# gorjanradevski/revisiting-spatial-temporal-layouts

Measured on AMD Instinct MI355X. Metric: clips/s STLT forward (T=32, N_obj=7, d=768), higher is better.
Workload: dtype f32; 1 GPU; cfg2: STLT forward, T=32, N=7, d=768, H=12, 4+8 layers, 174 classes; per_gpu_batch=1024, global_batch=1024, parallelism=batch-shard x1, no collective, cls_only_last_spatial=True

## Files before the change

revisiting-spatial-temporal-layouts_amd/csrc/gemm.hip:

```cpp
#include <cstdlib>
#include <type_traits>
#include "common.h"

namespace {

constexpr int BM = 256, BN = 128, BK = 32;
constexpr int GEMM_WAVES = 8;
constexpr int GEMM_LOADERS = 4;
constexpr int GEMM_THREADS = 64 * (GEMM_WAVES + GEMM_LOADERS);
constexpr int NSTAGE = 3;
constexpr int STAGE_FLOATS = (BM + BN) * BK;

typedef __attribute__((address_space(3))) void* lds_void_ptr;
typedef const __attribute__((address_space(1))) void* glb_void_ptr;

#ifndef STLT_GEMM_ABLATE
#define STLT_GEMM_ABLATE 0
#endif
__device__ __forceinline__ float half_wave_sum(float x) {
  x += __shfl_xor(x, 1, 64);
  x += __shfl_xor(x, 2, 64);
  x += __shfl_xor(x, 4, 64);
  x += __shfl_xor(x, 8, 64);
  x += __shfl_xor(x, 16, 64);
  return x;
}

struct SkPlan { int dp_rounds; int P[9]; int S[8]; };
struct SkNone {};
template <bool B, class T> auto karg(const T& t) { if constexpr (B) return t; else return SkNone{}; }

template <int ACT, bool STAMP, bool TA, bool TB, bool ADD, bool SK, bool GROUP = false>
__global__ __launch_bounds__(GEMM_THREADS, 3) void gemm_nt_kernel(const float* __restrict__ X, int64_t ldx,
                                                                  const float* __restrict__ W, int64_t ldw,
                                                                  const float* __restrict__ bias,
                                                                  const float* __restrict__ R, int64_t ldr,
                                                                  float* __restrict__ Y, int64_t ldy,
                                                                  int64_t slab_stride, int M, int N, int K,
                                                                  int tiles_m, int tiles_n, int n_split,
                                                                  float* __restrict__ partials,
                                                                  unsigned long long* __restrict__ dbg,
                                                                  const std::conditional_t<SK, SkPlan, SkNone> plan_in,
                                                                  const std::conditional_t<GROUP, StltGemmGroup, SkNone> grp_in,
                                                                  const std::conditional_t<ACT == STLT_ACT_GELU_BWD, StltGemmEpi, SkNone> epi_in) {
  SkPlan plan{}; StltGemmGroup grp{}; StltGemmEpi epi{};
  if constexpr (SK) plan = plan_in;
  if constexpr (GROUP) grp = grp_in;
  if constexpr (ACT == STLT_ACT_GELU_BWD) epi = epi_in;
  static_assert(!GROUP || SK, "grouped launches are stream-K launches");
  static_assert(ACT != STLT_ACT_GELU_BWD || (ADD && !GROUP), "the fused GELU backward reads u through the add-source");
  constexpr int NBIAS = 2;
  __shared__ __attribute__((aligned(16))) float smem[NSTAGE * STAGE_FLOATS + NBIAS * BN];

  const int tid = threadIdx.x;
  const int lane = tid & 63;
  const int wave = __builtin_amdgcn_readfirstlane(tid >> 6);
  const int wm = wave >> 1, wn = wave & 1;
  const int lr = lane & 31, lh = lane >> 5;
  const int nk_total = K / BK;
  int nk = GROUP ? 1 : nk_total / n_split;
  const int n_tiles = GROUP ? grp.tile_base[grp.n] : tiles_m * tiles_n * n_split;

  const int G = gridDim.x;
  int v = blockIdx.x;
  if ((G & 7) == 0) v = (blockIdx.x & 7) * (G >> 3) + (blockIdx.x >> 3);
  constexpr int GROUP_M = 4;
  const bool grouped = !SK && n_split == 1 && (G & 7) == 0;
  const int g_xcd = blockIdx.x & 7, g_local = blockIdx.x >> 3, g_gx = G >> 3;
  const int g_rounds = (n_tiles + G - 1) / G;
  int my_tiles, sk_first = 0, sk_kt0 = 0, sk_tail = 0;
  const bool hy = SK && plan.dp_rounds > 0;
  const int hy_R = hy ? plan.dp_rounds : 0;
  int hy_steps = 0;
  int g_p0 = 0, g_first = 0, g_nk_last = 1, g_total = 0;
  if constexpr (GROUP) {
    const int total = grp.step_base[grp.n];
    const int S = (total + G - 1) / G;
    const int s0 = v * S;
    if (s0 >= total) return;
    const int s1 = s0 + S < total ? s0 + S : total;
    while (grp.step_base[g_p0 + 1] <= s0) ++g_p0;
    const int nk0 = grp.p[g_p0].nk;
    const int lt0 = (s0 - grp.step_base[g_p0]) / nk0;
    sk_kt0 = s0 - grp.step_base[g_p0] - lt0 * nk0;
    g_first = grp.tile_base[g_p0] + lt0;
    int p1 = g_p0;
    while (grp.step_base[p1 + 1] <= s1 - 1) ++p1;
    g_nk_last = grp.p[p1].nk;
    const int lt1 = (s1 - 1 - grp.step_base[p1]) / g_nk_last;
    my_tiles = grp.tile_base[p1] + lt1 - g_first + 1;
    sk_tail = s1 - (grp.step_base[p1] + lt1 * g_nk_last);
    g_total = s1 - s0;
  } else
  if (hy) {
    const int e = plan.P[g_xcd + 1];
    const int s0 = plan.P[g_xcd] + g_local * plan.S[g_xcd];
    const int s1 = s0 + plan.S[g_xcd] < e ? s0 + plan.S[g_xcd] : e;
    int sk_tiles = 0;
    if (s0 < s1) {
      sk_first = s0 / nk;
      sk_kt0 = s0 - sk_first * nk;
      const int last = (s1 - 1) / nk;
      sk_tiles = last - sk_first + 1;
      sk_tail = s1 - last * nk;
      hy_steps = s1 - s0;
    }
    my_tiles = hy_R + sk_tiles;
  } else if (SK) {
    const int total = n_tiles * nk;
    const int S = (total + G - 1) / G;
    const int s0 = v * S;
    if (s0 >= total) return;
    const int s1 = s0 + S < total ? s0 + S : total;
    sk_first = s0 / nk;
    sk_kt0 = s0 - sk_first * nk;
// ... 183 lines not shown
      }
    }
  };
  if (wave >= GEMM_WAVES) {
    int l_it = 0, l_kt = kt_begin(0), l_stage = 0;
    bool l_fresh = true;
    auto l_step = [&]() {
      if ((STLT_GEMM_ABLATE & 32) ? l_fresh : (l_kt == 0 || l_fresh)) { dma_set_tile(l_it); l_fresh = false; }
      const int src_kt = (STLT_GEMM_ABLATE & 32) ? 0 : l_kt;
#pragma unroll
      for (int u = 0; u < NV; ++u) {
        issue_dma_part(0, src_kt, l_stage, u);
        issue_dma_part(1, src_kt, l_stage, u);
        issue_dma_part(2, src_kt, l_stage, u);
      }
      if (++l_kt == nk) { ++l_it; l_kt = kt_begin(l_it); if (!(STLT_GEMM_ABLATE & 32)) l_fresh = true; }
      if (++l_stage == NSTAGE) l_stage = 0;
    };
    dma_bias(0);
    l_step();
    if (total_steps > 1) {
      l_step();
      asm volatile("s_waitcnt vmcnt(12)" ::: "memory");
    } else {
      asm volatile("s_waitcnt vmcnt(0)" ::: "memory");
    }
    __builtin_amdgcn_s_barrier();
    int w_it = 0, w_kt = kt_begin(0);
    for (int step = 0; step < total_steps; ++step) {
      if (!GROUP && w_kt == nk - 1 && w_it + 1 < my_tiles) dma_bias(w_it + 1);
      if (!(STLT_GEMM_ABLATE & 1) && step + 2 < total_steps) {
        l_step();
        if (!(STLT_GEMM_ABLATE & 8)) asm volatile("s_waitcnt vmcnt(12)" ::: "memory");
      } else {
        asm volatile("s_waitcnt vmcnt(0)" ::: "memory");
      }
      __builtin_amdgcn_s_barrier();
      if (!GROUP && ++w_kt == nk) { ++w_it; w_kt = kt_begin(w_it); }
    }
    return;
  }
  f32x16 acc[2][2];
  auto init_acc = [&](int it, bool zero) {
    if (bias && !TB && !zero) {
      const float* src = bias_lds + (it & 1) * BN + wn * 64 + 4 * lh;
#pragma unroll
      for (int b = 0; b < 2; ++b)
#pragma unroll
        for (int q = 0; q < 4; ++q) {
          const f32x4 v = *reinterpret_cast<const f32x4*>(src + b * 32 + 8 * q);
#pragma unroll
          for (int j = 0; j < 4; ++j) { acc[0][b][4 * q + j] = v[j]; acc[1][b][4 * q + j] = v[j]; }
        }
    } else {
#pragma unroll
      for (int a = 0; a < 2; ++a)
#pragma unroll
        for (int b = 0; b < 2; ++b)
#pragma unroll
          for (int r = 0; r < 16; ++r) acc[a][b][r] = 0.f;
    }
  };

  auto mfma_chunk = [&](const Frags& f) {
#pragma unroll
    for (int e = 0; e < 4; ++e) {
      acc[0][0] = __builtin_amdgcn_mfma_f32_32x32x2f32(f.b0[e], f.a0[e], acc[0][0], 0, 0, 0);
      acc[0][1] = __builtin_amdgcn_mfma_f32_32x32x2f32(f.b1[e], f.a0[e], acc[0][1], 0, 0, 0);
      acc[1][0] = __builtin_amdgcn_mfma_f32_32x32x2f32(f.b0[e], f.a1[e], acc[1][0], 0, 0, 0);
      acc[1][1] = __builtin_amdgcn_mfma_f32_32x32x2f32(f.b1[e], f.a1[e], acc[1][1], 0, 0, 0);
    }
  };

  __builtin_amdgcn_s_barrier();
  init_acc(0, SK && !seg_complete(0));
  Frags fa = read_frags(0, 0), fb;

  int c_it = 0, c_kt = kt_begin(0);
  if constexpr (GROUP) nk = grp.p[g_p0].nk;
  int stage = 0;
  constexpr bool RES_PF = ADD && !SK && !TA && !TB;
  f32x4 rpf[RES_PF ? 8 : 1];
  bool rpf_ok = false;
  unsigned long long t_acc[6] = {0, 0, 0, 0, 0, 0}, t_prev = 0;
#define GSTAMP(k) do { if (STAMP) { __builtin_amdgcn_sched_barrier(0); unsigned long long t_now = __builtin_amdgcn_s_memtime(); __builtin_amdgcn_s_waitcnt(0xC07F); t_acc[k] += t_now - t_prev; t_prev = t_now; __builtin_amdgcn_sched_barrier(0); } } while (0)
  if (STAMP) { t_prev = __builtin_amdgcn_s_memtime(); __builtin_amdgcn_s_waitcnt(0xC07F); }
  for (int step = 0; step < total_steps; ++step) {
    const int next_stage = stage + 1 == NSTAGE ? 0 : stage + 1;
    if constexpr (RES_PF) {
      if (c_kt == nk - 1) {
        int m0, n0, split;
        tile_origin(c_it, m0, n0, split);
        rpf_ok = (m0 + BM <= M) && (n0 + BN <= N) && (ldr & 3) == 0 && ((uintptr_t)R & 15) == 0;
        if (rpf_ok) {
          const float* rrow = R + (int64_t)(m0 + wm * 64 + lr) * ldr + n0;
#pragma unroll
          for (int h = 0; h < 8; ++h) rpf[h] = *reinterpret_cast<const f32x4*>(rrow + wn * 64 + (h >> 2) * 32 + 8 * (h & 3) + 4 * lh);
        }
      }
    }
    fb = read_frags(stage, 1);
    mfma_chunk(fa);
    fa = read_frags(stage, 2);
    mfma_chunk(fb);
    fb = read_frags(stage, 3);
    mfma_chunk(fa);
    if (STAMP) asm volatile("" :: "v"(acc[0][0][0]), "v"(acc[1][1][15]));
    GSTAMP(0);
    asm volatile("s_waitcnt lgkmcnt(0)" ::: "memory");
    GSTAMP(1);
    __builtin_amdgcn_s_barrier();
    GSTAMP(2);
    GSTAMP(3);
    if (step + 1 < total_steps) fa = read_frags(next_stage, 0);
    mfma_chunk(fb);
    if (STAMP) asm volatile("" :: "v"(acc[0][0][0]), "v"(acc[1][1][15]));
    GSTAMP(4);
    stage = next_stage;

    if (++c_kt == nk || (SK && step == total_steps - 1)) {
      int m0, n0, split;
      tile_origin(c_it, m0, n0, split);
      if constexpr (GROUP) {
        int pi, lt;
        group_tile(c_it, pi, lt);
        Y = grp.p[pi].c; ldy = grp.p[pi].ldc; R = grp.p[pi].r; ldr = grp.p[pi].ldr; M = grp.p[pi].M; N = grp.p[pi].N;
      }
      float* Yt = Y + (int64_t)split * slab_stride;
      const bool partial = SK && !seg_complete(c_it);
      const bool vec_ok = (m0 + BM <= M) && (n0 + BN <= N) && (ldy & 3) == 0 && ((uintptr_t)Yt & 15) == 0 &&
                          (!ADD || ((ldr & 3) == 0 && ((uintptr_t)R & 15) == 0));
      auto t_row = [&](int a) { return TA ? wm * 64 + 2 * lr + a : wm * 64 + a * 32 + lr; };
      auto t_col4 = [&](int g) { return TB ? wn * 64 + 16 * (g >> 1) + 8 * lh + 4 * (g & 1) : wn * 64 + (g >> 2) * 32 + 8 * (g & 3) + 4 * lh; };
      auto group = [&](int a, int g) {
        f32x4 v;
#pragma unroll
        for (int j = 0; j < 4; ++j)
          v[j] = TB ? acc[a][j & 1][4 * (g >> 1) + 2 * (g & 1) + (j >> 1)] : acc[a][g >> 2][4 * (g & 3) + j];
        return v;
      };
      if (partial) {
        float* P = partials + (size_t)(2 * v + (c_it == hy_R ? 0 : 1)) * (BM * BN);
#pragma unroll
        for (int a = 0; a < 2; ++a)
#pragma unroll
          for (int g = 0; g < 8; ++g) *reinterpret_cast<f32x4*>(P + t_row(a) * BN + t_col4(g)) = group(a, g);
      } else if (ACT == STLT_ACT_GELU_BWD && vec_ok) {
        const uint64_t key = stlt_drop_key(epi.dr, epi.site);
        float* cs_row = epi.cs_part + ((size_t)(m0 / BM) * 16 + wm) * (size_t)N + n0;
        uint64_t drow[2];
#pragma unroll
        for (int a = 0; a < 2; ++a) drow[a] = epi.drop_rows ? (uint64_t)epi.drop_rows[m0 + t_row(a)] : (uint64_t)(m0 + t_row(a));
        constexpr int GB = 2;
#pragma unroll
        for (int hf = 0; hf < 8 / GB; ++hf) {
          f32x4 uv[2][GB];
#pragma unroll
          for (int a = 0; a < 2; ++a)
#pragma unroll
            for (int q = 0; q < GB; ++q) uv[a][q] = *reinterpret_cast<const f32x4*>(R + (int64_t)(m0 + t_row(a)) * ldr + n0 + t_col4(hf * GB + q));
#pragma unroll
          for (int q = 0; q < GB; ++q) {
            const int g = hf * GB + q;
            f32x4 cs = {0.f, 0.f, 0.f, 0.f};
#pragma unroll
            for (int a = 0; a < 2; ++a) {
              const f32x4 val = gelu_bwd4(group(a, g), uv[a][q], epi, key, drow[a] * (uint64_t)N + (uint64_t)(n0 + t_col4(g)));
              *reinterpret_cast<f32x4*>(Yt + (int64_t)(m0 + t_row(a)) * ldy + n0 + t_col4(g)) = val;
              cs += val;
            }
#pragma unroll
            for (int j = 0; j < 4; ++j) cs[j] = half_wave_sum(cs[j]);
            if (lr == 0) {
              *reinterpret_cast<f32x4*>(cs_row + t_col4(g)) = cs;
#pragma unroll
              for (int k = 1; k < 4; ++k) *reinterpret_cast<f32x4*>(cs_row + (size_t)(4 * k) * N + t_col4(g)) = f32x4{0.f, 0.f, 0.f, 0.f};
            }
          }
        }
      } else if (ACT == STLT_ACT_GELU_BWD) {
        const uint64_t key = stlt_drop_key(epi.dr, epi.site);
        float* cs_row = epi.cs_part + ((size_t)(m0 / BM) * 16 + wm) * (size_t)N;
#pragma unroll
        for (int g = 0; g < 8; ++g) {
          f32x4 cs = {0.f, 0.f, 0.f, 0.f};
          const int n = n0 + t_col4(g);
#pragma unroll
          for (int a = 0; a < 2; ++a) {
            const int m = m0 + t_row(a);
            const f32x4 acc4 = group(a, g);
            if (m < M) {
              const uint64_t drow1 = epi.drop_rows ? (uint64_t)epi.drop_rows[m] : (uint64_t)m;
#pragma unroll
              for (int j = 0; j < 4; ++j) {
                if (n + j < N) {
                  float v = acc4[j];
                  if (epi.dr.thr) v = stlt_keep_k(epi.dr.thr, key, drow1 * (uint64_t)N + (uint64_t)(n + j)) ? v * epi.dr.scale : 0.f;
                  v *= gelu_grad_epilogue(R[(int64_t)m * ldr + n + j]);
                  Yt[(int64_t)m * ldy + n + j] = v;
                  cs[j] += v;
                }
              }
            }
          }
#pragma unroll
          for (int j = 0; j < 4; ++j) cs[j] = half_wave_sum(cs[j]);
          if (lr == 0) {
#pragma unroll
            for (int j = 0; j < 4; ++j)
              if (n + j < N) {
                cs_row[n + j] = cs[j];
#pragma unroll
                for (int k = 1; k < 4; ++k) cs_row[(size_t)(4 * k) * N + n + j] = 0.f;
              }
          }
        }
      } else if (vec_ok) {
#pragma unroll
        for (int a = 0; a < 2; ++a) {
          const int m = m0 + t_row(a);
          float* yrow = Yt + (int64_t)m * ldy + n0;
          const float* rrow = ADD ? R + (int64_t)m * ldr + n0 : nullptr;
          constexpr int RB = 8;
          f32x4 rv[ADD ? RB : 1];
#pragma unroll
          for (int g = 0; g < 8; ++g) {
            if (ADD && g % RB == 0) {
              if (RES_PF && a == 0 && rpf_ok) {
#pragma unroll
                for (int h = 0; h < RB; ++h) rv[ADD ? h : 0] = rpf[RES_PF ? h : 0];
              } else {
#pragma unroll
                for (int h = 0; h < RB; ++h) rv[ADD ? h : 0] = *reinterpret_cast<const f32x4*>(rrow + t_col4(g + h));
              }
            }
            f32x4 val = group(a, g);
            if (ADD) val += rv[ADD ? g % RB : 0];
#pragma unroll
            for (int j = 0; j < 4; ++j) {
              if (ACT == STLT_ACT_GELU) val[j] = gelu_epilogue(val[j]);
              if (ACT == STLT_ACT_RELU) val[j] = fmaxf(val[j], 0.f);
            }
            if (STLT_GEMM_ABLATE & 16) asm volatile("" :: "v"(val));
            else *reinterpret_cast<f32x4*>(yrow + t_col4(g)) = val;
          }
        }
      } else {
#pragma unroll
        for (int a = 0; a < 2; ++a) {
          const int m = m0 + t_row(a);
#pragma unroll
          for (int g = 0; g < 8; ++g) {
            const int n = n0 + t_col4(g);
            const f32x4 val = group(a, g);
            float* yp = Yt + (int64_t)m * ldy + n;
            const float* rp = ADD ? R + (int64_t)m * ldr + n : nullptr;
#pragma unroll
            for (int j = 0; j < 4; ++j) {
              float x = val[j];
              if (m < M && n + j < N) {
                if (ADD) x += rp[j];
                if (ACT == STLT_ACT_GELU) x = gelu_epilogue(x);
                if (ACT == STLT_ACT_RELU) x = fmaxf(x, 0.f);
                yp[j] = x;
              }
            }
          }
        }
      }
      if (c_it + 1 < my_tiles) init_acc(c_it + 1, SK && !seg_complete(c_it + 1));
      ++c_it;
      c_kt = kt_begin(c_it);
      if constexpr (GROUP) {
        if (c_it < my_tiles) { int pi, lt; group_tile(c_it, pi, lt); nk = grp.p[pi].nk; }
      }
      GSTAMP(5);
    }
  }
  if (dbg && tid == 0) {
    dbg[4 * blockIdx.x + 1] = __builtin_amdgcn_s_memrealtime();
    dbg[4 * (size_t)gridDim.x + (size_t)gridDim.x * GEMM_WAVES * 6 + 1024 + 2 * blockIdx.x + 1] = __builtin_amdgcn_s_memtime();
  }
  if (STAMP && dbg && lane == 0) {
    unsigned long long* o = dbg + 4 * (size_t)gridDim.x + ((size_t)blockIdx.x * GEMM_WAVES + wave) * 6;
    for (int k = 0; k < 6; ++k) o[k] = t_acc[k];
  }
#undef GSTAMP
}


constexpr int FIXUP_CHUNKS = 16;
template <int ACT>
__global__ __launch_bounds__(256) void gemm_fixup_kernel(const float* __restrict__ partials, int S, int nk,
                                                         const float* __restrict__ bias, const float* __restrict__ R,
                                                         int64_t ldr, float* __restrict__ Y, int64_t ldy, int M, int N,
                                                         int tiles_m, int tiles_n, int G, const SkPlan plan, const StltGemmEpi epi) {
  __shared__ float cs_red[8][BN];
  const int t = blockIdx.x / FIXUP_CHUNKS, chunk = blockIdx.x - t * FIXUP_CHUNKS;
  const int lo = t * nk, hi = lo + nk;
  const bool hy = plan.dp_rounds > 0;
  const int gx = G >> 3;
  auto wg_of = [&](int s) {
    if (!hy) return s / S;
    int x = 0;
    while (x < 7 && s >= plan.P[x + 1]) ++x;
    return x * gx + (s - plan.P[x]) / plan.S[x];
  };
  auto start_of = [&](int v) {
    if (!hy) return v * S;
    const int x = v / gx;
    return plan.P[x] + (v - x * gx) * plan.S[x];
  };
  const int v_first = wg_of(lo), v_last = wg_of(hi - 1);
  if (v_first == v_last) return;
  int m0, n0;
  if (hy) {
    constexpr int GROUP_M = 4;
    const int p = plan.dp_rounds * G + t;
    const int band = p / (GROUP_M * tiles_n), w = p - band * (GROUP_M * tiles_n);
    const int rows = tiles_m - band * GROUP_M < GROUP_M ? tiles_m - band * GROUP_M : GROUP_M;
    const int tn_g = w / rows;
    m0 = (band * GROUP_M + (w - tn_g * rows)) * BM;
    n0 = tn_g * BN;
  } else {
    const int tm = t / tiles_n;
    m0 = tm * BM;
    n0 = (t - tm * tiles_n) * BN;
  }
  const int c4 = (threadIdx.x & 31) * 4;
  float bv[4];
#pragma unroll
  for (int e = 0; e < 4; ++e) bv[e] = (bias && n0 + c4 + e < N) ? bias[n0 + c4 + e] : 0.f;
  const int r_end = (chunk + 1) * (BM / FIXUP_CHUNKS);
  const uint64_t key = ACT == STLT_ACT_GELU_BWD ? stlt_drop_key(epi.dr, epi.site) : 0ull;
  f32x4 cs = {0.f, 0.f, 0.f, 0.f};
  for (int rr = chunk * (BM / FIXUP_CHUNKS) + (threadIdx.x >> 5); rr < r_end; rr += 8) {
    const int m = m0 + rr;
    if (m >= M) break;
    f32x4 acc = {0.f, 0.f, 0.f, 0.f};
    for (int v = v_first; v <= v_last; ++v) {
      if (hy && start_of(v) >= plan.P[v / gx + 1]) continue;
      const size_t slot = (size_t)(2 * v + (start_of(v) >= lo ? 0 : 1));
      acc += *reinterpret_cast<const f32x4*>(partials + slot * (BM * BN) + rr * BN + c4);
    }
    const uint64_t drow = (ACT == STLT_ACT_GELU_BWD && epi.drop_rows) ? (uint64_t)epi.drop_rows[m] : (uint64_t)m;
#pragma unroll
    for (int e = 0; e < 4; ++e) {
      const int n = n0 + c4 + e;
      if (n < N) {
        float val = acc[e] + bv[e];
        if (ACT == STLT_ACT_GELU_BWD) {
          if (epi.dr.thr) val = stlt_keep_k(epi.dr.thr, key, drow * (uint64_t)N + (uint64_t)n) ? val * epi.dr.scale : 0.f;
          val *= gelu_grad_epilogue(R[(int64_t)m * ldr + n]);
          cs[e] += val;
        } else if (R) {
          val += R[(int64_t)m * ldr + n];
        }
        if (ACT == STLT_ACT_GELU) val = gelu_epilogue(val);
        if (ACT == STLT_ACT_RELU) val = fmaxf(val, 0.f);
        Y[(int64_t)m * ldy + n] = val;
      }
    }
  }
  if (ACT == STLT_ACT_GELU_BWD) {
#pragma unroll
    for (int e = 0; e < 4; ++e) cs_red[threadIdx.x >> 5][c4 + e] = cs[e];
    __syncthreads();
    if (threadIdx.x < BN && n0 + (int)threadIdx.x < N) {
      float tsum = 0.f;
#pragma unroll
// ... 291 lines not shown
  if (act == STLT_ACT_GELU_BWD) {
    if (!epi_in || !epi.cs_part || !r || transA || (!transB && !on_copy) || n_split != 1 || bias)
      return stlt_set_error(STLT_EINVAL, "gemm: the fused GELU backward is the dX layout with u as the add-source and a column-sum buffer");
  }
  if (M < 0 || N <= 0 || K <= 0) return stlt_set_error(STLT_EINVAL, "gemm: bad shape (M=%lld N=%lld K=%lld)", (long long)M, (long long)N, (long long)K);
  const bool base_off = (((uintptr_t)a | (uintptr_t)b) & 15) != 0;
  if (K % BK != 0 || lda % 4 != 0 || ldb % 4 != 0 || base_off) {
    if ((n_split != 1 || act == STLT_ACT_GELU_BWD) && base_off && K % BK == 0 && lda % 4 == 0 && ldb % 4 == 0)
      return stlt_set_error(STLT_EINVAL, "gemm: a split product / the fused GELU backward needs %s 16-byte aligned", ((uintptr_t)a & 15) ? "a" : "b");
    if (n_split != 1 || act == STLT_ACT_GELU_BWD)
      return stlt_set_error(STLT_EINVAL, "gemm: a split product / the fused GELU backward needs K=%lld to be a multiple of %d and pitches that are multiples of 4", (long long)K, BK);
    return launch_gemm_any(transA, transB, a, lda, b, ldb, bias, r, ldr, c, ldc, M, N, K, act, s);
  }
  if (lda % 4 != 0 || ldb % 4 != 0 || (r && ldr < N) || ldc < N || lda < (transA ? M : K) || ldb < (transB ? N : K))
    return stlt_set_error(STLT_EINVAL, "gemm: bad leading dimension (lda=%lld ldb=%lld ldc=%lld)", (long long)lda, (long long)ldb, (long long)ldc);
  if (M > 0x7fffff00LL || N > 0x7fffff00LL || (bias && N > 0x3fffff00LL)) return stlt_set_error(STLT_EINVAL, "gemm: M/N too large");
  if (lda > 0x3fffffLL || ldb > 0x3fffffLL)
    return stlt_set_error(STLT_EINVAL, "gemm: row pitch too large (lda=%lld ldb=%lld, at most 4194303 floats)", (long long)lda, (long long)ldb);
  if (act != STLT_ACT_NONE && act != STLT_ACT_GELU && act != STLT_ACT_RELU && act != STLT_ACT_GELU_BWD) return stlt_set_error(STLT_EINVAL, "gemm: unknown activation %d", act);
  if (n_split < 1 || (K / BK) % n_split != 0) return stlt_set_error(STLT_EINVAL, "gemm: n_split=%d must divide K/32=%lld", n_split, (long long)(K / BK));
  if (transA && !transB) return stlt_set_error(STLT_EINVAL, "gemm: the (transA, !transB) layout is not built");
  if (n_split > 1 && (bias || act != STLT_ACT_NONE || r)) return stlt_set_error(STLT_EINVAL, "gemm: a split product takes no bias / activation / add-source");
  if ((transA || transB) && ((act != STLT_ACT_NONE && act != STLT_ACT_GELU_BWD) || bias)) return stlt_set_error(STLT_EINVAL, "gemm: bias/activation only with the forward (NT) layout");
  if (r && act != STLT_ACT_NONE && act != STLT_ACT_GELU_BWD) return stlt_set_error(STLT_EINVAL, "gemm: an add-source excludes an activation");
  if (M == 0) return 0;
  const int64_t tiles_m = (M + BM - 1) / BM, tiles_n = (N + BN - 1) / BN;
  if (tiles_m * tiles_n * n_split > 0x7fffffffLL) return stlt_set_error(STLT_EINVAL, "gemm: too many tiles");
  int64_t n_wg = tiles_m * tiles_n * n_split;
  if (n_wg > n_cu()) n_wg = n_cu();
  StltProfScope ps(STLT_K_GEMM, s);
  stlt_prof_add_flops(2.0 * (double)M * (double)N * (double)K);
  stlt_prof_note("gemm%s M=%lld N=%lld K=%lld act=%d%s tile=256x128 tiles=%lld", transA ? "(dW)" : (transB ? "(dX)" : (on_copy ? "(dX on the Wt copy)" : "")), (long long)M, (long long)N, (long long)K, act,
                 r ? "+R" : "", (long long)(tiles_m * tiles_n));
  const dim3 block(GEMM_THREADS);
  const int64_t n_tiles = tiles_m * tiles_n, nk = K / BK;
  const int64_t rounds = (n_tiles + n_cu() - 1) / n_cu();
  const double fill = (double)n_tiles / (double)(rounds * n_cu());
  static const double sk_fill = [] { const char* e = getenv("STLT_GEMM_SK_FILL"); return e ? atof(e) : 0.9; }();
  bool weighted = false;
  if (xcd_weights() && n_split == 1 && t_gemm_scratch && fill >= sk_fill && n_tiles >= 4 * (int64_t)n_cu() && n_tiles * nk < 0x7fffffffLL) {
    SkPlan probe{};
    int64_t tail = 0;
    weighted = make_sk_plan(n_tiles, nk, n_cu() < STLT_GEMM_SK_MAX_WG ? n_cu() : STLT_GEMM_SK_MAX_WG, xcd_weights(), true, probe, tail);
  }
  if (n_split == 1 && t_gemm_scratch && (fill < sk_fill || weighted) && n_tiles * nk < 0x7fffffffLL && !g_stlt_debug_buf) {
    int64_t G = n_cu() < STLT_GEMM_SK_MAX_WG ? n_cu() : STLT_GEMM_SK_MAX_WG;
    if (n_tiles * nk < 4 * G) G = (n_tiles * nk + 3) / 4;
    if (t_gemm_scratch_bytes >= (size_t)(2 * G) * BM * BN * sizeof(float)) {
      const int S = (int)((n_tiles * nk + G - 1) / G);
      dim3 grid((unsigned)G);
      float* P = t_gemm_scratch;
      stlt_prof_note("stream-K wg=%lld ksteps/wg=%d (+fix-up)", (long long)G, S);
      static const bool hybrid_on = [] { const char* e = getenv("STLT_GEMM_HYBRID"); return e ? atoi(e) != 0 : true; }();
      SkPlan plan{};
      int64_t fix_tiles = n_tiles;
      if (hybrid_on && G == n_cu()) {
        int64_t tail = 0;
        if (make_sk_plan(n_tiles, nk, G, xcd_weights(), weighted, plan, tail)) fix_tiles = tail;
        else plan = SkPlan{};
      }
#define LAUNCH_SK(ACTV, TAV, TBV, ADDV) hipLaunchKernelGGL((gemm_nt_kernel<ACTV, false, TAV, TBV, ADDV, true>), grid, block, 0, s, a, lda, b, ldb, bias, r, ldr, c, ldc, slab_stride, (int)M, (int)N, (int)K, (int)tiles_m, (int)tiles_n, 1, P, nullptr, plan, SkNone{}, karg<(ACTV) == STLT_ACT_GELU_BWD>(epi))
      if (transA) { if (r) LAUNCH_SK(STLT_ACT_NONE, true, true, true); else LAUNCH_SK(STLT_ACT_NONE, true, true, false); }
      else if (transB && act == STLT_ACT_GELU_BWD) LAUNCH_SK(STLT_ACT_GELU_BWD, false, true, true);
      else if (transB) { if (r) LAUNCH_SK(STLT_ACT_NONE, false, true, true); else LAUNCH_SK(STLT_ACT_NONE, false, true, false); }
      else if (act == STLT_ACT_GELU_BWD) LAUNCH_SK(STLT_ACT_GELU_BWD, false, false, true);
      else if (r) LAUNCH_SK(STLT_ACT_NONE, false, false, true);
      else if (act == STLT_ACT_GELU) LAUNCH_SK(STLT_ACT_GELU, false, false, false);
      else if (act == STLT_ACT_RELU) LAUNCH_SK(STLT_ACT_RELU, false, false, false);
      else LAUNCH_SK(STLT_ACT_NONE, false, false, false);
#undef LAUNCH_SK
      if (int e = stlt_check_launch("gemm_nt_kernel(stream-k)")) return e;
      dim3 fgrid((unsigned)(fix_tiles * FIXUP_CHUNKS)), fblock(256);
#define FIX(ACTV) hipLaunchKernelGGL((gemm_fixup_kernel<ACTV>), fgrid, fblock, 0, s, P, S, (int)nk, bias, r, ldr, c, ldc, (int)M, (int)N, (int)tiles_m, (int)tiles_n, (int)G, plan, epi)
      if (act == STLT_ACT_GELU_BWD) FIX(STLT_ACT_GELU_BWD);
      else if (act == STLT_ACT_GELU) FIX(STLT_ACT_GELU);
      else if (act == STLT_ACT_RELU) FIX(STLT_ACT_RELU);
      else FIX(STLT_ACT_NONE);
#undef FIX
      return stlt_check_launch("gemm_fixup_kernel");
    }
  }
  dim3 grid((unsigned)n_wg);
  stlt_prof_note("wg=%lld rounds=%lld ksteps=%lld split=%d", (long long)n_wg, (long long)((tiles_m * tiles_n * n_split + n_wg - 1) / n_wg), (long long)(nk / n_split), n_split);
#define LAUNCH(ACTV, STAMPV, TAV, TBV, ADDV) hipLaunchKernelGGL((gemm_nt_kernel<ACTV, STAMPV, TAV, TBV, ADDV, false>), grid, block, 0, s, a, lda, b, ldb, bias, r, ldr, c, ldc, slab_stride, (int)M, (int)N, (int)K, (int)tiles_m, (int)tiles_n, n_split, (float*)nullptr, g_stlt_debug_buf, SkNone{}, SkNone{}, karg<(ACTV) == STLT_ACT_GELU_BWD>(epi))
  if (transA) { if (r) LAUNCH(STLT_ACT_NONE, false, true, true, true); else LAUNCH(STLT_ACT_NONE, false, true, true, false); }
  else if (transB && act == STLT_ACT_GELU_BWD) LAUNCH(STLT_ACT_GELU_BWD, false, false, true, true);
  else if (transB) { if (r) LAUNCH(STLT_ACT_NONE, false, false, true, true); else LAUNCH(STLT_ACT_NONE, false, false, true, false); }
  else if (act == STLT_ACT_GELU_BWD) LAUNCH(STLT_ACT_GELU_BWD, false, false, false, true);
  else if (r && g_stlt_debug_buf && getenv("STLT_GEMM_STAMP")) LAUNCH(STLT_ACT_NONE, true, false, false, true);
  else if (r) LAUNCH(STLT_ACT_NONE, false, false, false, true);
  else if (g_stlt_debug_buf && getenv("STLT_GEMM_STAMP")) LAUNCH(STLT_ACT_NONE, true, false, false, false);
  else if (act == STLT_ACT_GELU) LAUNCH(STLT_ACT_GELU, false, false, false, false);
  else if (act == STLT_ACT_RELU) LAUNCH(STLT_ACT_RELU, false, false, false, false);
  else LAUNCH(STLT_ACT_NONE, false, false, false, false);
#undef LAUNCH
  return stlt_check_launch("gemm_nt_kernel");
}

bool stlt_gemm_has_scratch() { return t_gemm_scratch != nullptr && t_gemm_scratch_bytes >= STLT_GEMM_SCRATCH_BYTES; }
float* stlt_gemm_scratch_ptr(size_t* bytes) { *bytes = t_gemm_scratch ? t_gemm_scratch_bytes : 0; return t_gemm_scratch; }

int launch_weight_grad_group(const StltWeightGradItem* items, int n_items, hipStream_t s) {
  if (!items || n_items < 1 || n_items > STLT_GEMM_GROUP_MAX) return stlt_set_error(STLT_EINVAL, "weight_grad_group: 1..%d items", STLT_GEMM_GROUP_MAX);
  if (!stlt_gemm_has_scratch()) return stlt_set_error(STLT_EWORKSPACE, "weight_grad_group: no stream-K scratch lent (StltGemmScratch)");
  StltGemmGroup grp{};
  int64_t tiles = 0, steps = 0;
  double flops = 0.0;
  int n = 0;
  for (int i = 0; i < n_items; ++i) {
    const StltWeightGradItem& it = items[i];
    if (!it.g_w || it.rows == 0) continue;
    if (!it.dy || !it.x || it.n_out <= 0 || it.k_in <= 0 || it.rows < 0 || it.rows % BK != 0 || it.n_out % 4 != 0 || it.k_in % 4 != 0)
      return stlt_set_error(STLT_EINVAL, "weight_grad_group: item %d: rows=%lld must be a multiple of %d, n_out=%lld / k_in=%lld multiples of 4", i,
                            (long long)it.rows, BK, (long long)it.n_out, (long long)it.k_in);
    if (it.n_out > 0x3fffffLL || it.k_in > 0x3fffffLL || it.rows > 0x7fffff00LL) return stlt_set_error(STLT_EINVAL, "weight_grad_group: item too large");
    if (const char* off = stlt_first_unaligned16({{"dy", it.dy}, {"x", it.x}}))
      return stlt_set_error(STLT_EINVAL, "weight_grad_group: item %d: %s must be 16-byte aligned", i, off);
    const int64_t tm = (it.n_out + BM - 1) / BM, tn = (it.k_in + BN - 1) / BN;
    StltGemmProblem& q = grp.p[n];
    q.a = it.dy; q.lda = (int)it.n_out; q.b = it.x; q.ldb = (int)it.k_in; q.r = it.g_w; q.ldr = (int)it.k_in; q.c = it.g_w; q.ldc = (int)it.k_in;
    q.M = (int)it.n_out; q.N = (int)it.k_in; q.nk = (int)(it.rows / BK); q.tiles_n = (int)tn;
    grp.tile_base[n] = (int)tiles;
    grp.step_base[n] = (int)steps;
    tiles += tm * tn;
    steps += tm * tn * (it.rows / BK);
    if (tiles > 0x3fffffffLL || steps > 0x3fffffffLL) return stlt_set_error(STLT_EINVAL, "weight_grad_group: too many k-steps");
    flops += 2.0 * (double)it.n_out * (double)it.k_in * (double)it.rows;
    ++n;
  }
  if (n == 0) return 0;
  grp.n = n;
  for (int i = n; i <= STLT_GEMM_GROUP_MAX; ++i) { grp.tile_base[i] = (int)tiles; grp.step_base[i] = (int)steps; }
  int64_t G = n_cu() < STLT_GEMM_SK_MAX_WG ? n_cu() : STLT_GEMM_SK_MAX_WG;
  if (steps < 4 * G) G = (steps + 3) / 4;
  const int S = (int)((steps + G - 1) / G);
  StltProfScope ps(STLT_K_GEMM, s);
  stlt_prof_add_flops(flops);
  stlt_prof_note("gemm(dW group) products=%d tiles=%lld ksteps=%lld tile=256x128 stream-K wg=%lld ksteps/wg=%d (+fix-up)", n, (long long)tiles, (long long)steps, (long long)G, S);
  float* P = t_gemm_scratch;
  hipLaunchKernelGGL((gemm_nt_kernel<STLT_ACT_NONE, false, true, true, true, true, true>), dim3((unsigned)G), dim3(GEMM_THREADS), 0, s,
                     (const float*)nullptr, (int64_t)0, (const float*)nullptr, (int64_t)0, (const float*)nullptr, (const float*)nullptr, (int64_t)0,
                     (float*)nullptr, (int64_t)0, (int64_t)0, 0, 0, BK, 0, 0, 1, P, (unsigned long long*)nullptr, SkPlan{}, grp, SkNone{});
  if (int e = stlt_check_launch("gemm_nt_kernel(grouped stream-k)")) return e;
  hipLaunchKernelGGL(gemm_fixup_group_kernel, dim3((unsigned)(tiles * FIXUP_CHUNKS)), dim3(256), 0, s, P, S, grp);
  return stlt_check_launch("gemm_fixup_group_kernel");
}

StltGemmScratch::StltGemmScratch(void* p, size_t bytes) : prev_(t_gemm_scratch), prev_bytes_(t_gemm_scratch_bytes) {
  t_gemm_scratch = static_cast<float*>(p);
  t_gemm_scratch_bytes = p ? bytes : 0;
}
StltGemmScratch::~StltGemmScratch() {
  t_gemm_scratch = prev_;
  t_gemm_scratch_bytes = prev_bytes_;
}
StltGemmWgCap::StltGemmWgCap(int n) : prev_(t_gemm_wg_cap) { t_gemm_wg_cap = n > 0 ? (n + 7) / 8 * 8 : 0; }
StltGemmWgCap::~StltGemmWgCap() { t_gemm_wg_cap = prev_; }
void stlt_gemm_set_scratch_impl(void* p, size_t bytes) {
  t_gemm_scratch = static_cast<float*>(p);
  t_gemm_scratch_bytes = p ? bytes : 0;
}

int launch_reduce_slabs(const float* slabs, int64_t stride, int n_slabs, float* dst, int64_t n, int accumulate, hipStream_t s) {
  if (!slabs || !dst || n_slabs < 1) return stlt_set_error(STLT_EINVAL, "reduce_slabs: bad arguments");
  if (n == 0) return 0;
  if (accumulate) { int err = 0; if (reduce_defer_take(slabs, stride, n_slabs, dst, nullptr, nullptr, 1, n, s, &err)) return err; }
  const bool off16 = (((uintptr_t)slabs | (uintptr_t)dst) & 15) != 0 || (n_slabs > 1 && stride % 4 != 0);
  if (off16 && (n + 15) / 16 > 0x7fffffffLL) return stlt_set_error(STLT_EINVAL, "reduce_slabs: n=%lld is too large for slabs / dst off a 16-byte boundary", (long long)n);
  if ((n_slabs > 32 && n <= 16384) || off16) {
    stlt_prof_note("reduce n=%lld slabs=%d tall blocks=%lld", (long long)n, n_slabs, (long long)((n + 15) / 16));
    hipLaunchKernelGGL(reduce_tall_kernel, dim3((unsigned)((n + 15) / 16)), dim3(256), 0, s, slabs, stride, n_slabs, dst, n, accumulate);
    return stlt_check_launch("reduce_tall_kernel");
  }
  int64_t blocks = (n + 1023) / 1024;
  if (blocks > 2048) blocks = 2048;
  stlt_prof_note("reduce n=%lld slabs=%d blocks=%lld", (long long)n, n_slabs, (long long)blocks);
  hipLaunchKernelGGL(reduce_slabs_kernel, dim3((unsigned)blocks), dim3(256), 0, s, slabs, stride, n_slabs, dst, n, accumulate);
  return stlt_check_launch("reduce_slabs_kernel");
// ... 41 lines not shown
```

Baseline: 9901 clips/s.

## Overlap GEMM epilogue stores with next tile's MFMA at tile boundaries

Adds a skewed boundary path for forward whole-tile GEMM launches. The last k-step of a tile and the first k-step of the next are merged, so the epilogue (bias/residual add, activation, stores) of each accumulator half is interleaved with MFMAs of the other half. Scheduling group barriers pin the instruction order for some variants. The aim is to hide the serial epilogue cost between tiles, at the price of much more complex control flow, register pressure from residual prefetch, and 32-bit address arithmetic limits. It also extends the timestamp instrumentation with per-epilogue counters.

```diff
diff --git a/revisiting-spatial-temporal-layouts_amd/csrc/gemm.hip b/revisiting-spatial-temporal-layouts_amd/csrc/gemm.hip
--- a/revisiting-spatial-temporal-layouts_amd/csrc/gemm.hip
+++ b/revisiting-spatial-temporal-layouts_amd/csrc/gemm.hip
@@ -14,6 +14,9 @@
 typedef __attribute__((address_space(3))) void* lds_void_ptr;
 typedef const __attribute__((address_space(1))) void* glb_void_ptr;
 
+#ifndef STLT_GEMM_NOPIPE
+#define STLT_GEMM_NOPIPE 0
+#endif
 #ifndef STLT_GEMM_ABLATE
 #define STLT_GEMM_ABLATE 0
 #endif
@@ -30,7 +33,7 @@
 struct SkNone {};
 template <bool B, class T> auto karg(const T& t) { if constexpr (B) return t; else return SkNone{}; }
 
-template <int ACT, bool STAMP, bool TA, bool TB, bool ADD, bool SK, bool GROUP = false>
+template <int ACT, bool STAMP, bool TA, bool TB, bool ADD, bool SK, bool GROUP = false, bool SKW = false>
 __global__ __launch_bounds__(GEMM_THREADS, 3) void gemm_nt_kernel(const float* __restrict__ X, int64_t ldx,
                                                                   const float* __restrict__ W, int64_t ldw,
                                                                   const float* __restrict__ bias,
@@ -380,13 +383,222 @@
   constexpr bool RES_PF = ADD && !SK && !TA && !TB;
   f32x4 rpf[RES_PF ? 8 : 1];
   bool rpf_ok = false;
-  unsigned long long t_acc[6] = {0, 0, 0, 0, 0, 0}, t_prev = 0;
-#define GSTAMP(k) do { if (STAMP) { __builtin_amdgcn_sched_barrier(0); unsigned long long t_now = __builtin_amdgcn_s_memtime(); __builtin_amdgcn_s_waitcnt(0xC07F); t_acc[k] += t_now - t_prev; t_prev = t_now; __builtin_amdgcn_sched_barrier(0); } } while (0)
-  if (STAMP) { t_prev = __builtin_amdgcn_s_memtime(); __builtin_amdgcn_s_waitcnt(0xC07F); }
+  unsigned t_acc[6] = {0, 0, 0, 0, 0, 0}, t_prev = 0;
+#define GSTAMP(k) do { if (STAMP) { __builtin_amdgcn_sched_barrier(0); const unsigned t_now = (unsigned)__builtin_amdgcn_s_memtime(); __builtin_amdgcn_s_waitcnt(0xC07F); t_acc[k] += t_now - t_prev; t_prev = t_now; __builtin_amdgcn_sched_barrier(0); } } while (0)
+  if (STAMP) { t_prev = (unsigned)__builtin_amdgcn_s_memtime(); __builtin_amdgcn_s_waitcnt(0xC07F); }
+  unsigned t_epi[4] = {0, 0, 0, 0};
+#define ESTAMP(k) do { if (STAMP) { __builtin_amdgcn_sched_barrier(0); const unsigned t_now = (unsigned)__builtin_amdgcn_s_memtime(); __builtin_amdgcn_s_waitcnt(0xC07F); t_acc[5] += t_now - t_prev; t_epi[k] += t_now - t_prev; t_prev = t_now; __builtin_amdgcn_sched_barrier(0); } } while (0)
+  static_assert(!SKW || (!TA && !TB && !SK && !GROUP && ACT != STLT_ACT_GELU_BWD), "boundary steps: forward layout, whole-tile launches");
+  constexpr bool SKEW = SKW, skew = SKW;
+  bool pend = false;
+  char* y_pend = nullptr;
+  const char* r_pend = nullptr;
+  const uint32_t y_lane = ((uint32_t)(wm * 64 + lr) * (uint32_t)ldy + (uint32_t)(wn * 64 + 4 * lh)) * 4u;
+  const uint32_t r_lane = ADD ? ((uint32_t)(wm * 64 + lr) * (uint32_t)ldr + (uint32_t)(wn * 64 + 4 * lh)) * 4u : 0u;
+  struct Half { f32x4 a, b0, b1; };
+  auto read_half = [&](int stg, int c, int a) __attribute__((always_inline)) {
+    const float* s = smem + stg * STAGE_FLOATS;
+    const int off = ((2 * c + lh) ^ sw) * 4;
+    Half h;
+    h.a = *reinterpret_cast<const f32x4*>(s + a_row + a * 32 * BK + off);
+    h.b0 = *reinterpret_cast<const f32x4*>(s + b_row + off);
+    h.b1 = *reinterpret_cast<const f32x4*>(s + b_row + 32 * BK + off);
+    return h;
+  };
+  auto init_half = [&](int a, int it) __attribute__((always_inline)) {
+    if (bias) {
+      const float* src = bias_lds + (it & 1) * BN + wn * 64 + 4 * lh;
+#pragma unroll
+      for (int b = 0; b < 2; ++b)
+#pragma unroll
+        for (int q = 0; q < 4; ++q) {
+          const f32x4 v = *reinterpret_cast<const f32x4*>(src + b * 32 + 8 * q);
+#pragma unroll
+          for (int j = 0; j < 4; ++j) acc[a][b][4 * q + j] = v[j];
+        }
+    } else {
+#pragma unroll
+      for (int b = 0; b < 2; ++b)
+#pragma unroll
+        for (int r = 0; r < 16; ++r) acc[a][b][r] = 0.f;
+    }
+  };
+  auto gcol = [](int g) { return (g >> 2) * 32 + 8 * (g & 3); };
+  auto finish = [&](float x) {
+    if (ACT == STLT_ACT_GELU) x = gelu_epilogue(x);
+    if (ACT == STLT_ACT_RELU) x = fmaxf(x, 0.f);
+    return x;
+  };
+  auto bchunk = [&](int a_mf, const Half& h, auto DRAIN, int a_dr, int c, char* yrow, auto RELOAD, const char* rnext) __attribute__((always_inline)) {
+    f32x4 out;
+#pragma unroll
+    for (int e = 0; e < 4; ++e) {
+#pragma unroll
+      for (int b = 0; b < 2; ++b) {
+        acc[a_mf][b] = __builtin_amdgcn_mfma_f32_32x32x2f32(b ? h.b1[e] : h.b0[e], h.a[e], acc[a_mf][b], 0, 0, 0);
+        if constexpr (decltype(DRAIN)::value) {
+          const int v = 2 * e + b, g = 2 * c + (v >> 2), j = v & 3;
+          float x = acc[a_dr][g >> 2][4 * (g & 3) + j];
+          if (ADD) x += rpf[RES_PF ? g : 0][j];
+          out[j] = finish(x);
+          if (j == 3) {
+            if (STLT_GEMM_ABLATE & 16) asm volatile("" :: "v"(out));
+            else *reinterpret_cast<f32x4*>(yrow + y_lane + gcol(g) * 4) = out;
+            if constexpr (ADD && decltype(RELOAD)::value) {
+              if (g < 4) rpf[RES_PF ? g : 0] = *reinterpret_cast<const f32x4*>(rnext + r_lane + gcol(g) * 4);
+            }
+          }
+        }
+      }
+    }
+  };
+  constexpr int NVAL = ACT == STLT_ACT_GELU ? 24 : (ADD || ACT == STLT_ACT_RELU) ? 1 : 0;
+  constexpr bool PIN = STLT_GEMM_NOPIPE == 2 || (STLT_GEMM_NOPIPE == 0 && !ADD && ACT != STLT_ACT_GELU);
+#define PIPE_ONE(RL, ST) do { if (!PIN) break; __builtin_amdgcn_sched_group_barrier(0x008, 1, 0); if constexpr (NVAL > 0) __builtin_amdgcn_sched_group_barrier(0x002, NVAL > 0 ? NVAL : 1, 0); \
+    if (ST) { __builtin_amdgcn_sched_group_barrier(0x040, 1, 0); if constexpr (ADD && (RL)) __builtin_amdgcn_sched_group_barrier(0x020, 1, 0); } } while (0)
+#define PIPE_CHUNK(NR, RL) do { if (!PIN) break; __builtin_amdgcn_sched_group_barrier(0x100, NR, 0); PIPE_ONE(RL, 0); PIPE_ONE(RL, 0); PIPE_ONE(RL, 0); PIPE_ONE(RL, 1); \
+    PIPE_ONE(RL, 0); PIPE_ONE(RL, 0); PIPE_ONE(RL, 0); PIPE_ONE(RL, 1); } while (0)
+  auto boundary = [&](auto PEND, auto LAST, int step, int next_stage) __attribute__((always_inline)) {
+    constexpr bool P = decltype(PEND)::value, L = decltype(LAST)::value;
+    constexpr std::bool_constant<(P && L)> RL_A{};
+    constexpr std::bool_constant<L> RL_B{};
+    char* y0 = nullptr;
+    const char* r0 = nullptr;
+    if constexpr (L) {
+      int m0, n0, split;
+      tile_origin(c_it, m0, n0, split);
+      y0 = reinterpret_cast<char*>(Y + (int64_t)m0 * ldy + n0);
+      if constexpr (ADD) {
+        r0 = reinterpret_cast<const char*>(R + (int64_t)m0 * ldr + n0);
+        if constexpr (!P) {
+#pragma unroll
+          for (int g = 0; g < 8; ++g) rpf[RES_PF ? g : 0] = *reinterpret_cast<const f32x4*>(r0 + r_lane + gcol(g) * 4);
+        }
+      }
+    }
+    if constexpr (ADD && P && !L) {
+#pragma unroll
+      for (int g = 4; g < 8; ++g) rpf[RES_PF ? g : 0] = *reinterpret_cast<const f32x4*>(r_pend + r_lane + gcol(g) * 4);
+    }
+    Half h0, h1;
+    h0.a = fa.a0; h0.b0 = fa.b0; h0.b1 = fa.b1;
+    h1 = read_half(stage, 1, 0);
+    bchunk(0, h0, PEND, 1, 0, y_pend, RL_A, r0);
+    h0 = read_half(stage, 2, 0);
+    bchunk(0, h1, PEND, 1, 1, y_pend, RL_A, r0);
+    h1 = read_half(stage, 3, 0);
+    bchunk(0, h0, PEND, 1, 2, y_pend, RL_A, r0);
+    h0 = read_half(stage, 0, 1);
+    bchunk(0, h1, PEND, 1, 3, y_pend, RL_A, r0);
+    if constexpr (P) {
+      if constexpr (PIN && ADD && !L) __builtin_amdgcn_sched_group_barrier(0x020, 4, 0);
+      PIPE_CHUNK(3, P && L); PIPE_CHUNK(3, P && L); PIPE_CHUNK(3, false); PIPE_CHUNK(3, false);
+    }
+    __builtin_amdgcn_sched_barrier(0);
+    if constexpr (P) init_half(1, c_it);
+    const char* r1 = (ADD && L) ? r0 + (int64_t)32 * ldr * 4 : nullptr;
+    h1 = read_half(stage, 1, 1);
+    bchunk(1, h0, LAST, 0, 0, y0, RL_B, r1);
+    h0 = read_half(stage, 2, 1);
+    bchunk(1, h1, LAST, 0, 1, y0, RL_B, r1);
+    h1 = read_half(stage, 3, 1);
+    bchunk(1, h0, LAST, 0, 2, y0, RL_B, r1);
+    if constexpr (L) { PIPE_CHUNK(3, L); PIPE_CHUNK(3, L); PIPE_CHUNK(3, false); }
+    __builtin_amdgcn_sched_barrier(0);
+    asm volatile("s_waitcnt lgkmcnt(0)" ::: "memory");
+    __builtin_amdgcn_s_barrier();
+    if (step + 1 < total_steps) {
+      if constexpr (L) {
+        const Half n = read_half(next_stage, 0, 0);
+        fa.a0 = n.a; fa.b0 = n.b0; fa.b1 = n.b1;
+      } else {
+        fa = read_frags(next_stage, 0);
+      }
+    }
+    bchunk(1, h1, LAST, 0, 3, y0, RL_B, r1);
+    if constexpr (L) { PIPE_CHUNK(4, false); }
+    __builtin_amdgcn_sched_barrier(0);
+    if constexpr (L) {
+      if (c_it + 1 < my_tiles) {
+        init_half(0, c_it + 1);
+        pend = true;
+        y_pend = y0 + (int64_t)32 * ldy * 4;
+        r_pend = r1;
+      } else {
+        pend = false;
+        if constexpr (ADD) {
+#pragma unroll
+          for (int g = 4; g < 8; ++g) rpf[RES_PF ? g : 0] = *reinterpret_cast<const f32x4*>(r1 + r_lane + gcol(g) * 4);
+        }
+#pragma unroll
+        for (int g = 0; g < 8; ++g) {
+          f32x4 out;
+#pragma unroll
+          for (int j = 0; j < 4; ++j) {
+            float x = acc[1][g >> 2][4 * (g & 3) + j];
+            if (ADD) x += rpf[RES_PF ? g : 0][j];
+            out[j] = finish(x);
+          }
+          if (STLT_GEMM_ABLATE & 16) asm volatile("" :: "v"(out));
+          else *reinterpret_cast<f32x4*>(y0 + (int64_t)32 * ldy * 4 + y_lane + gcol(g) * 4) = out;
+        }
+      }
+      ++c_it;
+      c_kt = 0;
+    } else {
+      pend = false;
+      ++c_kt;
+    }
+    if (STAMP) asm volatile("" :: "v"(acc[0][0][0]), "v"(acc[1][1][15]));
+    ESTAMP(P && L ? 2 : L ? 0 : 1);
+  };
+#undef PIPE_CHUNK
+#undef PIPE_ONE
+  if constexpr (SKW) {
+    int step = 0;
+    for (int it = 0; it < my_tiles; ++it) {
+      int n_int = nk - 1;
+      if (it > 0) {
+        const int next_stage = stage + 1 == NSTAGE ? 0 : stage + 1;
+        boundary(std::true_type{}, std::false_type{}, step, next_stage);
+        stage = next_stage;
+        ++step;
+        n_int = nk - 2;
+      }
+      for (int i = 0; i < n_int; ++i, ++step) {
+        const int next_stage = stage + 1 == NSTAGE ? 0 : stage + 1;
+        fb = read_frags(stage, 1);
+        mfma_chunk(fa);
+        fa = read_frags(stage, 2);
+        mfma_chunk(fb);
+        fb = read_frags(stage, 3);
+        mfma_chunk(fa);
+        if (STAMP) asm volatile("" :: "v"(acc[0][0][0]), "v"(acc[1][1][15]));
+        GSTAMP(0);
+        asm volatile("s_waitcnt lgkmcnt(0)" ::: "memory");
+        GSTAMP(1);
+        __builtin_amdgcn_s_barrier();
+        GSTAMP(2);
+        GSTAMP(3);
+        fa = read_frags(next_stage, 0);
+        mfma_chunk(fb);
+        if (STAMP) asm volatile("" :: "v"(acc[0][0][0]), "v"(acc[1][1][15]));
+        GSTAMP(4);
+        stage = next_stage;
+        ++c_kt;
+      }
+      {
+        const int next_stage = stage + 1 == NSTAGE ? 0 : stage + 1;
+        boundary(std::false_type{}, std::true_type{}, step, next_stage);
+        stage = next_stage;
+        ++step;
+      }
+    }
+  } else
   for (int step = 0; step < total_steps; ++step) {
     const int next_stage = stage + 1 == NSTAGE ? 0 : stage + 1;
     if constexpr (RES_PF) {
-      if (c_kt == nk - 1) {
+      if (c_kt == nk - 1 && !skew) {
         int m0, n0, split;
         tile_origin(c_it, m0, n0, split);
         rpf_ok = (m0 + BM <= M) && (n0 + BN <= N) && (ldr & 3) == 0 && ((uintptr_t)R & 15) == 0;
@@ -416,7 +628,8 @@
     GSTAMP(4);
     stage = next_stage;
 
-    if (++c_kt == nk || (SK && step == total_steps - 1)) {
+    ++c_kt;
+    if (!SKW && (c_kt == nk || (SK && step == total_steps - 1))) {
       int m0, n0, split;
       tile_origin(c_it, m0, n0, split);
       if constexpr (GROUP) {
@@ -513,6 +726,44 @@
               }
           }
         }
+      } else if (STAMP && vec_ok) {
+#pragma unroll
+        for (int a = 0; a < 2; ++a) {
+          const int m = m0 + t_row(a);
+          float* yrow = Yt + (int64_t)m * ldy + n0;
+#pragma unroll
+          for (int hb = 0; hb < 2; ++hb) {
+            f32x4 rv[ADD ? 4 : 1];
+            if constexpr (ADD) {
+              const float* rrow = R + (int64_t)m * ldr + n0;
+              if (RES_PF && a == 0 && rpf_ok) {
+#pragma unroll
+                for (int h = 0; h < 4; ++h) rv[h] = rpf[RES_PF ? 4 * hb + h : 0];
+              } else {
+#pragma unroll
+                for (int h = 0; h < 4; ++h) rv[h] = *reinterpret_cast<const f32x4*>(rrow + t_col4(4 * hb + h));
+              }
+              __builtin_amdgcn_s_waitcnt(0x0070);
+            }
+            ESTAMP(0);
+#pragma unroll
+            for (int g = 4 * hb; g < 4 * hb + 4; ++g)
+#pragma unroll
+              for (int j = 0; j < 4; ++j) {
+                float x = acc[a][g >> 2][4 * (g & 3) + j];
+                if (ADD) x += rv[ADD ? g & 3 : 0][j];
+                if (ACT == STLT_ACT_GELU) x = gelu_epilogue(x);
+                if (ACT == STLT_ACT_RELU) x = fmaxf(x, 0.f);
+                acc[a][g >> 2][4 * (g & 3) + j] = x;
+              }
+#pragma unroll
+            for (int i = 0; i < 16; ++i) asm volatile("" :: "v"(acc[a][hb][i]));
+            ESTAMP(1);
+          }
+#pragma unroll
+          for (int g = 0; g < 8; ++g) *reinterpret_cast<f32x4*>(yrow + t_col4(g)) = group(a, g);
+          ESTAMP(2);
+        }
       } else if (vec_ok) {
 #pragma unroll
         for (int a = 0; a < 2; ++a) {
@@ -567,6 +818,8 @@
         }
       }
       if (c_it + 1 < my_tiles) init_acc(c_it + 1, SK && !seg_complete(c_it + 1));
+      if (STAMP) asm volatile("" :: "v"(acc[0][0][0]), "v"(acc[1][1][15]));
+      ESTAMP(3);
       ++c_it;
       c_kt = kt_begin(c_it);
       if constexpr (GROUP) {
@@ -582,8 +835,13 @@
   if (STAMP && dbg && lane == 0) {
     unsigned long long* o = dbg + 4 * (size_t)gridDim.x + ((size_t)blockIdx.x * GEMM_WAVES + wave) * 6;
     for (int k = 0; k < 6; ++k) o[k] = t_acc[k];
+    if (blockIdx.x < 32) {
+      unsigned long long* e = dbg + 4 * (size_t)gridDim.x + (size_t)gridDim.x * GEMM_WAVES * 6 + ((size_t)blockIdx.x * GEMM_WAVES + wave) * 4;
+      for (int k = 0; k < 4; ++k) e[k] = t_epi[k];
+    }
   }
 #undef GSTAMP
+#undef ESTAMP
 }
 
 
@@ -1041,18 +1299,26 @@
   }
   dim3 grid((unsigned)n_wg);
   stlt_prof_note("wg=%lld rounds=%lld ksteps=%lld split=%d", (long long)n_wg, (long long)((tiles_m * tiles_n * n_split + n_wg - 1) / n_wg), (long long)(nk / n_split), n_split);
-#define LAUNCH(ACTV, STAMPV, TAV, TBV, ADDV) hipLaunchKernelGGL((gemm_nt_kernel<ACTV, STAMPV, TAV, TBV, ADDV, false>), grid, block, 0, s, a, lda, b, ldb, bias, r, ldr, c, ldc, slab_stride, (int)M, (int)N, (int)K, (int)tiles_m, (int)tiles_n, n_split, (float*)nullptr, g_stlt_debug_buf, SkNone{}, SkNone{}, karg<(ACTV) == STLT_ACT_GELU_BWD>(epi))
+  static const bool boundary_on = [] { const char* e = getenv("STLT_GEMM_BOUNDARY"); return !(e && e[0] == '0'); }();
+  const bool skw = boundary_on && !transA && !transB && n_split == 1 && act != STLT_ACT_GELU_BWD && nk >= 2 && M % BM == 0 && N % BN == 0 && ldc % 4 == 0 &&
+                   ((uintptr_t)c & 15) == 0 && ldc <= 0x3fffffLL && (!r || (ldr % 4 == 0 && ldr <= 0x3fffffLL && ((uintptr_t)r & 15) == 0));
+#define LAUNCH_(ACTV, STAMPV, TAV, TBV, ADDV, SKWV) hipLaunchKernelGGL((gemm_nt_kernel<ACTV, STAMPV, TAV, TBV, ADDV, false, false, SKWV>), grid, block, 0, s, a, lda, b, ldb, bias, r, ldr, c, ldc, slab_stride, (int)M, (int)N, (int)K, (int)tiles_m, (int)tiles_n, n_split, (float*)nullptr, g_stlt_debug_buf, SkNone{}, SkNone{}, karg<(ACTV) == STLT_ACT_GELU_BWD>(epi))
+#define LAUNCH(ACTV, STAMPV, TAV, TBV, ADDV) LAUNCH_(ACTV, STAMPV, TAV, TBV, ADDV, false)
+#define LAUNCH_FWD(ACTV, STAMPV, ADDV) do { if (skw) LAUNCH_(ACTV, STAMPV, false, false, ADDV, true); else LAUNCH_(ACTV, STAMPV, false, false, ADDV, false); } while (0)
   if (transA) { if (r) LAUNCH(STLT_ACT_NONE, false, true, true, true); else LAUNCH(STLT_ACT_NONE, false, true, true, false); }
   else if (transB && act == STLT_ACT_GELU_BWD) LAUNCH(STLT_ACT_GELU_BWD, false, false, true, true);
   else if (transB) { if (r) LAUNCH(STLT_ACT_NONE, false, false, true, true); else LAUNCH(STLT_ACT_NONE, false, false, true, false); }
   else if (act == STLT_ACT_GELU_BWD) LAUNCH(STLT_ACT_GELU_BWD, false, false, false, true);
-  else if (r && g_stlt_debug_buf && getenv("STLT_GEMM_STAMP")) LAUNCH(STLT_ACT_NONE, true, false, false, true);
-  else if (r) LAUNCH(STLT_ACT_NONE, false, false, false, true);
-  else if (g_stlt_debug_buf && getenv("STLT_GEMM_STAMP")) LAUNCH(STLT_ACT_NONE, true, false, false, false);
-  else if (act == STLT_ACT_GELU) LAUNCH(STLT_ACT_GELU, false, false, false, false);
-  else if (act == STLT_ACT_RELU) LAUNCH(STLT_ACT_RELU, false, false, false, false);
-  else LAUNCH(STLT_ACT_NONE, false, false, false, false);
+  else if (r && g_stlt_debug_buf && getenv("STLT_GEMM_STAMP")) LAUNCH_FWD(STLT_ACT_NONE, true, true);
+  else if (act == STLT_ACT_GELU && g_stlt_debug_buf && getenv("STLT_GEMM_STAMP")) LAUNCH_FWD(STLT_ACT_GELU, true, false);
+  else if (r) LAUNCH_FWD(STLT_ACT_NONE, false, true);
+  else if (g_stlt_debug_buf && getenv("STLT_GEMM_STAMP")) LAUNCH_FWD(STLT_ACT_NONE, true, false);
+  else if (act == STLT_ACT_GELU) LAUNCH_FWD(STLT_ACT_GELU, false, false);
+  else if (act == STLT_ACT_RELU) LAUNCH_FWD(STLT_ACT_RELU, false, false);
+  else LAUNCH_FWD(STLT_ACT_NONE, false, false);
+#undef LAUNCH_FWD
 #undef LAUNCH
+#undef LAUNCH_
   return stlt_check_launch("gemm_nt_kernel");
 }
 
```

Result: no change. 9961 clips/s (median of 6 runs) (+0.6%).
